# annikabrundyn/driving-dirty

Hardware: AMD Instinct MI355X
Metric: 6-view scenes/sec fwd+bwd, roadmap model bs=32 (higher is better)
Workload: dtype f32

## Files before the change

### driving-dirty_amd/csrc/conv3x3.hip

```cpp
#include <stdlib.h>

#include "dd_common.h"

namespace {

constexpr int EPI_BIAS_RELU_BITS = 5;
constexpr int EPI_RELU_BITS = 6;
constexpr int EPI_BIAS_STATS = 7;
constexpr int EPI_RELU_MASK_AFF = 8;
constexpr int EPI_RELU_BITS_W1 = 9;


template <int CIN, int S>
struct StripCfg {
  static constexpr int PXB = CIN * 4;
  static constexpr int CHUNKS = CIN / 4;
  static constexpr int NPX = 32 * S + 2;
  static constexpr int SLOTB = NPX * PXB;
  static constexpr int NCH = NPX * CHUNKS;
  static constexpr int NLOAD = (NCH + 63) / 64;
  static constexpr int SPILLB = (NLOAD * 64 - NCH) * 16;
  static constexpr int WAVEB = 3 * SLOTB + SPILLB;
  static constexpr int KGROUPS = (CIN == 32) ? 36 : 5;
  static constexpr int WFLOATS = KGROUPS * 64 * 4;
};

template <int CIN>
__device__ __forceinline__ int swz(int q) {
  return CIN == 32 ? ((q >> 1) & 7) : 0;
}

template <int CIN, int S>
__device__ __forceinline__ void load_row(const float* __restrict__ img, int H, int W, int iy, int gx0, int lane,
                                         f32x4 (&r)[StripCfg<CIN, S>::NLOAD]) {
  using C = StripCfg<CIN, S>;
  const bool rowok = (iy >= 0) && (iy < H);
  const __amdgpu_buffer_rsrc_t rs = dd_rsrc(img + (long)(rowok ? iy : 0) * W * CIN, rowok ? W * C::PXB : 0);
#pragma unroll
  for (int i = 0; i < C::NLOAD; ++i) {
    const int c = lane + 64 * i;
    const int q = c / C::CHUNKS, ch = c % C::CHUNKS;
    const int off = (c < C::NCH) ? ((gx0 + q) * C::PXB + ch * 16) : -16;
    r[i] = dd_bload4<DD_AUX_NT>(rs, off);
  }
}

template <int CIN, int S>
__device__ __forceinline__ void load_row_img(const float* __restrict__ img, int H, int W, int iy, int gx0, int lane,
                                             f32x4 (&r)[StripCfg<CIN, S>::NLOAD]) {
  using C = StripCfg<CIN, S>;
  const bool rowok = (iy >= 0) && (iy < H);
  const int so = rowok ? iy * W * C::PXB : 0;
  const __amdgpu_buffer_rsrc_t rs = dd_rsrc(img, rowok ? so + W * C::PXB : 0);
#pragma unroll
  for (int i = 0; i < C::NLOAD; ++i) {
    const int c = lane + 64 * i;
    const int q = c / C::CHUNKS, ch = c % C::CHUNKS;
    const int off = (c < C::NCH) ? ((gx0 + q) * C::PXB + ch * 16) : -16;
    r[i] = dd_bload4<DD_AUX_NT>(rs, off, so);
  }
}

template <int CIN, int S, bool SWZ>
__device__ __forceinline__ void store_row(char* slot, char* spill, int lane,
                                          const f32x4 (&r)[StripCfg<CIN, S>::NLOAD]) {
  using C = StripCfg<CIN, S>;
#pragma unroll
  for (int i = 0; i < C::NLOAD; ++i) {
    const int c = lane + 64 * i;
    const int q = c / C::CHUNKS, ch = c % C::CHUNKS;
    char* dst = slot + q * C::PXB + ((ch ^ (SWZ ? swz<CIN>(q) : 0)) << 4);
    if (64 * (i + 1) > C::NCH) dst = (c < C::NCH) ? dst : spill + (c - C::NCH) * 16;
    *(f32x4*)dst = r[i];
  }
}

template <int S, bool SWZ>
__device__ __forceinline__ void store_row_aff(char* slot, char* spill, int lane, const f32x4 (&r)[StripCfg<32, S>::NLOAD],
                                              bool rowok, int gx0, int W, f32x4 sc, f32x4 sh) {
  using C = StripCfg<32, S>;
#pragma unroll
  for (int i = 0; i < C::NLOAD; ++i) {
    const int c = lane + 64 * i;
    const int q = c / C::CHUNKS, ch = c % C::CHUNKS;
    char* dst = slot + q * C::PXB + ((ch ^ (SWZ ? swz<32>(q) : 0)) << 4);
    if (64 * (i + 1) > C::NCH) dst = (c < C::NCH) ? dst : spill + (c - C::NCH) * 16;
    const bool in = rowok && (gx0 + q >= 0) && (gx0 + q < W);
    f32x4 v = r[i];
    v.x = in ? fmaxf(v.x * sc.x + sh.x, 0.f) : 0.f;
    v.y = in ? fmaxf(v.y * sc.y + sh.y, 0.f) : 0.f;
    v.z = in ? fmaxf(v.z * sc.z + sh.z, 0.f) : 0.f;
    v.w = in ? fmaxf(v.w * sc.w + sh.w, 0.f) : 0.f;
    *(f32x4*)dst = v;
  }
}

template <int CIN, int S, int EPI, int WPB, bool AFF = false>
__global__ __launch_bounds__(WPB * 64) void conv_strip_fwd(const float* __restrict__ x, const float* __restrict__ wp,
                                                           const float* __restrict__ bias,
                                                           const float* __restrict__ msk, float* __restrict__ y,
                                                           unsigned* __restrict__ bits_out, int B, int H, int W, int Ho,
                                                           int Wo, int nstrips, const float* __restrict__ aff = nullptr,
                                                           float* __restrict__ stats = nullptr) {
  using C = StripCfg<CIN, S>;
  extern __shared__ __attribute__((aligned(16))) char smem[];
  const int tid = threadIdx.x;
  const int lane = tid & 63;
  const int wave = __builtin_amdgcn_readfirstlane(tid >> 6);
  {
    f32x4* wl4 = (f32x4*)smem;
    const f32x4* wg4 = (const f32x4*)wp;
    for (int i = tid; i < C::WFLOATS / 4; i += WPB * 64) wl4[i] = wg4[i];
  }
  __syncthreads();
  char* ring = smem + C::WFLOATS * 4 + wave * C::WAVEB;
  char* spill = ring + 3 * C::SLOTB;
  const char* wl = smem;
  const int h = lane >> 5, n = lane & 31;
  const float bv = (EPI == DD_EPI_BIAS || EPI == DD_EPI_BIAS_RELU || EPI == EPI_BIAS_RELU_BITS || EPI == EPI_BIAS_STATS) ? bias[n] : 0.f;
  f32x4 asc = {1.f, 1.f, 1.f, 1.f}, ash = {0.f, 0.f, 0.f, 0.f};
  if (AFF) {
// ... 70 lines not shown
#pragma unroll
        for (int jp = 0; jp < 5; ++jp) {
          const int tap = min(2 * jp + h, 8);
          const int dy = tap / 3, dx = tap - 3 * dy;
          const char* rowb = ring + ((S * yy + dy) % 3) * C::SLOTB;
          const f32x4 a = *(const f32x4*)(rowb + (S * n + dx) * 16);
          const f32x4 w = *(const f32x4*)(wl + (jp * 64 + lane) * 16);
          acc = DD_MFMA(a.x, w.x, acc);
          acc = DD_MFMA(a.y, w.y, acc);
          acc = DD_MFMA(a.z, w.z, acc);
        }
      }

#pragma unroll
      for (int s = 0; s < S; ++s) {
        const int iy = S * yy + 2 + s;
        if constexpr (AFF) store_row_aff<S, true>(ring + ((iy + 1) % 3) * C::SLOTB, spill, lane, pre[s], iy >= 0 && iy < H, gx0, W, asc, ash);
        else store_row<CIN, S, true>(ring + ((iy + 1) % 3) * C::SLOTB, spill, lane, pre[s]);
      }

      const __amdgpu_buffer_rsrc_t ys = dd_rsrc(y + orow, Wo * 128);
      unsigned sign_word = 0;
#pragma unroll
      for (int r = 0; r < 16; ++r) {
        float v = acc[r];
        if (EPI == DD_EPI_BIAS || EPI == EPI_BIAS_STATS) v += bv;
        if (EPI == EPI_BIAS_STATS && x0 + dd_acc_row(r, lane) < Wo) {
          st_sum += v;
          st_sq += v * v;
        }
        if (EPI == DD_EPI_BIAS_RELU || EPI == EPI_BIAS_RELU_BITS) v = fmaxf(v + bv, 0.f);
        if (EPI == DD_EPI_RELU_MASK) v = (mreg[r] > 0.f) ? v : 0.f;
        if (EPI == EPI_RELU_MASK_AFF) v = (mreg[r] * msc + msh > 0.f) ? v : 0.f;
        if (EPI == EPI_RELU_BITS) v = ((__builtin_bit_cast(unsigned, mreg[r]) >> n) & 1u) ? v : 0.f;
        dd_bstore1<DD_AUX_NT>(ys, ((x0 + dd_acc_row(r, lane)) * 32 + n) * 4, v);
        if (EPI == EPI_BIAS_RELU_BITS) {
          const unsigned long long m = __ballot(v > 0.f);
          const int i0 = (r & 3) + 8 * (r >> 2);
          if (n == i0) sign_word = (unsigned)m;
          if (n == i0 + 4) sign_word = (unsigned)(m >> 32);
        }
      }
      if (EPI == EPI_BIAS_RELU_BITS) {
        const __amdgpu_buffer_rsrc_t bs = dd_rsrc(bits_out + (long)(b * Ho + yy) * Wo, Wo * 4);
        __builtin_amdgcn_raw_buffer_store_b32(sign_word, bs, (h == 0) ? (x0 + n) * 4 : -16, 0, 0);
      }
    }
  }
  if (EPI == EPI_BIAS_STATS) {
    const long gwl = ((long)(blockIdx.x * WPB + wave) * 64 + lane) * 2;
    stats[gwl] = st_sum;
    stats[gwl + 1] = st_sq;
  }
}

template <int WPB, int MASK>
__global__ __launch_bounds__(WPB * 64) void conv_s2_dgrad(const float* __restrict__ dy, const float* __restrict__ wp,
                                                          const float* __restrict__ msk, float* __restrict__ dx,
                                                          int B, int H, int W, int Ho, int Wo, int nstrips,
                                                          const float* __restrict__ aff = nullptr) {
  using C = StripCfg<32, 1>;
  extern __shared__ __attribute__((aligned(16))) char smem[];
  const int tid = threadIdx.x;
  const int lane = tid & 63;
  const int wave = __builtin_amdgcn_readfirstlane(tid >> 6);
  {
    f32x4* wl4 = (f32x4*)smem;
    const f32x4* wg4 = (const f32x4*)wp;
    for (int i = tid; i < C::WFLOATS / 4; i += WPB * 64) wl4[i] = wg4[i];
  }
  __syncthreads();
  const int nr = (H + 1) / 2;
  const float msc = (MASK == 3) ? aff[64 + (lane & 31)] : 1.f, msh = (MASK == 3) ? aff[96 + (lane & 31)] : 0.f;
  char* ring = smem + C::WFLOATS * 4 + wave * C::WAVEB;
  char* spill = ring + 3 * C::SLOTB;
  const char* wl = smem;
  const int h = lane >> 5, n = lane & 31;

  long idx, end;
  dd_range((long)B * nstrips * nr, blockIdx.x * WPB + wave, gridDim.x * WPB, idx, end);
  while (idx < end) {
    const long col = idx / nr;
    const int r0 = (int)(idx - col * nr);
    const int r1 = (int)min((long)nr, r0 + (end - idx));
    idx += r1 - r0;
    const int b = (int)(col / nstrips), s0 = (int)(col % nstrips) * 32;
    const float* dyb = dy + (long)b * Ho * Wo * 32;

#pragma unroll
    for (int d = 0; d < 2; ++d) {
      f32x4 t[C::NLOAD];
      load_row<32, 1>(dyb, Ho, Wo, r0 + d, s0, lane, t);
      store_row<32, 1, true>(ring + ((r0 + d) % 3) * C::SLOTB, spill, lane, t);
    }

    for (int r = r0; r < r1; ++r) {
      f32x4 pre[C::NLOAD];
      load_row<32, 1>(dyb, Ho, Wo, r + 2, s0, lane, pre);
      __builtin_amdgcn_sched_barrier(0);

      const char* row_r = ring + (r % 3) * C::SLOTB;
      const char* row_r1 = ring + ((r + 1) % 3) * C::SLOTB;
#define DD_TILE(PY, PX, NTAP, ...)                                                              \
  {                                                                                             \
    constexpr int taps[NTAP][3] = {__VA_ARGS__};                                                \
    const int yi = 2 * r + (PY);                                                                \
// ... 113 lines not shown
      float anext[16];
      {
        const bool ok = yy + 1 < Ho;
        const __amdgpu_buffer_rsrc_t as = dd_rsrc(dyb + (long)(ok ? yy + 1 : 0) * Wo * 32, ok ? Wo * 128 : 0);
#pragma unroll
        for (int pp = 0; pp < 16; ++pp) anext[pp] = dd_bload1<DD_AUX_NT>(as, aoff + pp * 256);
      }
      __builtin_amdgcn_sched_barrier(0);

      if (CIN == 32) {
        const char* rb0 = ring + ((S * yy + 0) % 3) * C::SLOTB;
        const char* rb1 = ring + ((S * yy + 1) % 3) * C::SLOTB;
        const char* rb2 = ring + ((S * yy + 2) % 3) * C::SLOTB;
#pragma unroll
        for (int pp = 0; pp < 16; ++pp) {
          const float a = areg[pp];
          bsum += a;
          const int off = (S * (2 * pp + h)) * 128 + n * 4;
#pragma unroll
          for (int dx = 0; dx < 3; ++dx) {
            acc[0 + dx] = DD_MFMA(a, *(const float*)(rb0 + off + dx * 128), acc[0 + dx]);
            acc[3 + dx] = DD_MFMA(a, *(const float*)(rb1 + off + dx * 128), acc[3 + dx]);
            acc[6 + dx] = DD_MFMA(a, *(const float*)(rb2 + off + dx * 128), acc[6 + dx]);
          }
        }
      } else {
        const char* rb = ring + ((S * yy + dy4) % 3) * C::SLOTB + dx4 * 16 + c4 * 4;
#pragma unroll
        for (int pp = 0; pp < 16; ++pp) {
          const float a = areg[pp];
          bsum += a;
          acc[0] = DD_MFMA(a, *(const float*)(rb + (S * (2 * pp + h)) * 16), acc[0]);
        }
      }

#pragma unroll
      for (int s = 0; s < S; ++s) {
        const int iy = S * yy + 2 + s;
        if constexpr (AFF) store_row_aff<S, false>(ring + ((iy + 1) % 3) * C::SLOTB, spill, lane, pre[s], iy >= 0 && iy < H, gx0, W, asc, ash);
        else store_row<CIN, S, false>(ring + ((iy + 1) % 3) * C::SLOTB, spill, lane, pre[s]);
      }
#pragma unroll
      for (int pp = 0; pp < 16; ++pp) areg[pp] = anext[pp];
    }
  }

#pragma unroll
  for (int t = 0; t < NT; ++t)
#pragma unroll
    for (int r = 0; r < 16; ++r) part[(((long)gw * NT + t) * 16 + r) * 64 + lane] = acc[t][r];
  bpart[(long)gw * 64 + lane] = bsum;
}

template <int CIN>
__global__ __launch_bounds__(1024) void conv_wgrad_reduce(const float* __restrict__ part,
                                                          const float* __restrict__ bpart, float* __restrict__ dw,
                                                          float* __restrict__ db, int nw) {
  constexpr int NT = (CIN == 32) ? 9 : 1;
  constexpr int G = 16;
  __shared__ double red[G][64];
  const int l = threadIdx.x & 63, g = threadIdx.x >> 6;
  const int row = blockIdx.x;
  const float* src = (row < NT * 16) ? part + (long)row * 64 + l : bpart + l;
  const long stride = (row < NT * 16) ? (long)NT * 16 * 64 : 64;
  double s0 = 0.0, s1 = 0.0, s2 = 0.0, s3 = 0.0;
  int w = g;
  for (; w + 3 * G < nw; w += 4 * G) {
    s0 += (double)src[(long)w * stride];
    s1 += (double)src[(long)(w + G) * stride];
    s2 += (double)src[(long)(w + 2 * G) * stride];
    s3 += (double)src[(long)(w + 3 * G) * stride];
  }
  for (; w < nw; w += G) s0 += (double)src[(long)w * stride];
  red[g][l] = (s0 + s1) + (s2 + s3);
  __syncthreads();
  if (g != 0) return;
  double sd = 0.0;
#pragma unroll
  for (int i = 0; i < G; ++i) sd += red[i][l];
  const float s = (float)sd;
  if (row < NT * 16) {
    const int t = row >> 4, r = row & 15;
    const int o = dd_acc_row(r, l), j = l & 31;
    if (CIN == 32) {
      dw[((long)o * 32 + j) * 9 + t] = s;
    } else if (j < 27) {
      dw[((long)o * 3 + (j % 3)) * 9 + (j / 3)] = s;
    }
  } else {
    const double other = __shfl_xor(sd, 32);
    if (l < 32) db[l] = (float)(sd + other);
  }
}

__global__ void conv_pack_kernel(const float* __restrict__ w, float* __restrict__ p, int cin_real, int kind) {
  const int idx = blockIdx.x * blockDim.x + threadIdx.x;
  if (cin_real == 32) {
    if (idx >= 36 * 64 * 4) return;
    const int i = idx & 3, lane = (idx >> 2) & 63, g = idx >> 8;
    const int j = g & 3, t = g >> 2;
    const int n = lane & 31, c = 8 * j + 4 * (lane >> 5) + i;
    float v;
    if (kind == 0) v = w[((long)n * 32 + c) * 9 + t];
    else if (kind == 1) v = w[((long)c * 32 + n) * 9 + (8 - t)];
    else v = w[((long)c * 32 + n) * 9 + t];
    p[idx] = v;
  } else {
    if (idx >= 5 * 64 * 4) return;
    const int i = idx & 3, lane = (idx >> 2) & 63, jp = idx >> 8;
    const int n = lane & 31, tap = 2 * jp + (lane >> 5);
    p[idx] = (tap < 9 && i < 3) ? w[((long)n * 3 + i) * 9 + tap] : 0.f;
  }
}

constexpr int WINO_UFLOATS = 3 * 4 * 2 * 2 * 64 * 4;

__device__ __forceinline__ f32x2 pk_sub2(f32x2 a, f32x2 b) {
// ... 1314 lines not shown
    if (xx >= 1 && xx <= W && yy >= 1 && yy <= H) {
      const f32x4 g = *(const f32x4*)(dy + ((b * H + (yy - 1)) * W + (xx - 1)) * dy_cstore + dy_coff + 4 * q);
      const unsigned m = bits_pad[pp] >> (4 * q);
      o.x = (m & 1u) ? g.x : 0.f;
      o.y = (m & 2u) ? g.y : 0.f;
      o.z = (m & 4u) ? g.z : 0.f;
      o.w = (m & 8u) ? g.w : 0.f;
    }
    __builtin_nontemporal_store(o, out_pad + i);
  }
}

__global__ void relu_bwd_kernel(const f32x4* __restrict__ dy, const f32x4* __restrict__ y, f32x4* __restrict__ out,
                                long n4) {
  for (long i = (long)blockIdx.x * blockDim.x + threadIdx.x; i < n4; i += (long)gridDim.x * blockDim.x) {
    const f32x4 g = dy[i], v = y[i];
    f32x4 o;
    o.x = v.x > 0.f ? g.x : 0.f;
    o.y = v.y > 0.f ? g.y : 0.f;
    o.z = v.z > 0.f ? g.z : 0.f;
    o.w = v.w > 0.f ? g.w : 0.f;
    out[i] = o;
  }
}

int check_desc(const dd_conv_desc* d) {
  DD_REQUIRE(d != nullptr, DD_ERR_BAD_ARG, "conv: NULL descriptor");
  DD_REQUIRE(d->batch > 0 && d->height > 0 && d->width > 0, DD_ERR_BAD_ARG, "conv: non-positive size");
  DD_REQUIRE(d->ksize == 3 && d->pad == 1, DD_ERR_UNSUPPORTED, "conv: only k3 p1 is implemented (got k%d p%d)", d->ksize, d->pad);
  DD_REQUIRE(d->stride == 1 || d->stride == 2, DD_ERR_UNSUPPORTED, "conv: stride %d", d->stride);
  DD_REQUIRE(d->cout == 32, DD_ERR_UNSUPPORTED, "conv: Cout %d (only 32)", d->cout);
  DD_REQUIRE((d->cin_real == 32 && d->cin_store == 32) || (d->cin_real == 3 && d->cin_store == 4), DD_ERR_UNSUPPORTED,
             "conv: Cin %d stored as %d (supported: 32/32, 3/4)", d->cin_real, d->cin_store);
  DD_REQUIRE(!(d->cin_real == 3 && d->stride == 2), DD_ERR_UNSUPPORTED, "conv: Cin 3 with stride 2");
  DD_REQUIRE((long)d->width * 128 < (1L << 31), DD_ERR_UNSUPPORTED, "conv: row too long for a 32-bit buffer descriptor");
  return 0;
}

int resident_grid(const dd_conv_desc* d, long row_tiles, int wpb, int per_cu) {
  long blocks = (long)dd_cu_budget_internal() * per_cu;
  if (d->rows_per_task > 0) blocks = min(blocks, max(1L, row_tiles / d->rows_per_task / wpb));
  return (int)max(1L, min(blocks, (row_tiles + wpb - 1) / wpb));
}

template <int CIN, int S, int EPI, int WPB, bool AFF = false>
int launch_fwd(const float* x, const float* wp, const float* bias, const float* msk, float* y, const dd_conv_desc* d,
               hipStream_t st, unsigned* bits_out = nullptr, const float* aff = nullptr, float* stats = nullptr) {
  using C = StripCfg<CIN, S>;
  const int Ho = dd_conv_out(d->height, S), Wo = dd_conv_out(d->width, S);
  const int nstrips = (Wo + 31) / 32;
  const size_t lds = C::WFLOATS * 4 + (size_t)WPB * C::WAVEB;
  const int per_cu = (int)max((size_t)1, min((size_t)2, (size_t)(160 * 1024) / lds));
  const int grid = resident_grid(d, (long)d->batch * nstrips * Ho, WPB, per_cu);
  auto k = conv_strip_fwd<CIN, S, EPI, WPB, AFF>;
  if (int rc = dd_allow_lds((const void*)k, lds)) return rc;
  hipLaunchKernelGGL(k, dim3(grid), dim3(WPB * 64), lds, st, x, wp, bias, msk, y, bits_out, d->batch, d->height, d->width,
                     Ho, Wo, nstrips, aff, stats);
  DD_LAUNCH_CHECK("conv_strip_fwd");
  return 0;
}

template <int MASK>
int launch_s2_dgrad(const float* dy, const float* packed_dgrad, const float* relu_src, float* dx, const dd_conv_desc* d, hipStream_t st,
                    const float* aff) {
  using C = StripCfg<32, 1>;
  constexpr int WPB = 8;
  const int H = d->height, W = d->width, Ho = dd_conv_out(H, 2), Wo = dd_conv_out(W, 2);
  const int ns = (W + 1) / 2, nr = (H + 1) / 2;
  const int nstrips = (ns + 31) / 32;
  const size_t lds = C::WFLOATS * 4 + (size_t)WPB * C::WAVEB;
  const int grid = resident_grid(d, (long)d->batch * nstrips * nr, WPB, 1);
  auto k = conv_s2_dgrad<WPB, MASK>;
  if (int rc = dd_allow_lds((const void*)k, lds)) return rc;
  hipLaunchKernelGGL(k, dim3(grid), dim3(WPB * 64), lds, st, dy, packed_dgrad, relu_src, dx, d->batch, H, W, Ho, Wo, nstrips, aff);
  DD_LAUNCH_CHECK("conv_s2_dgrad");
  return 0;
}

template <int EPI>
int launch_wino2(const float* x, const float* up, const float* bias, const unsigned* bits_in, float* y, unsigned* bits_out,
                 const dd_conv_desc* d, hipStream_t st, const float* x4 = nullptr, float* w1part = nullptr, int* nw_out = nullptr) {
  using C = StripCfg<32, 1>;
  using C4 = StripCfg<4, 1>;
  constexpr int WPB = 4;
  const int nstrips = (d->width + 31) / 32;
  static const bool ring_env = getenv("DD_WINO2_RING") != nullptr;
  static const bool ring_w1 = getenv("DD_WINO2_RING_W1") != nullptr;
  const bool ring = ring_env || (EPI == EPI_RELU_BITS_W1 && ring_w1);
  DD_REQUIRE((long)d->height * d->width * 128 < (1L << 30), DD_ERR_UNSUPPORTED, "conv_wino2: image of %d x %d pixels: the kernel addresses an image with 30-bit offsets",
             d->height, d->width);
  const size_t lds = (size_t)WINO2_UFLOATS * 4 + (ring ? (size_t)WPB * (4 * C::SLOTB + C::SPILLB) : 0) +
                     (EPI == EPI_RELU_BITS_W1 ? (size_t)WPB * (4 * C4::SLOTB + C4::SPILLB) + 128 : 0);
  const int grid = resident_grid(d, (long)d->batch * nstrips * ((d->height + 1) / 2), WPB, 1);
  if (nw_out) *nw_out = grid * WPB;
  if (int rc = dd_allow_lds(ring ? (const void*)conv_wino2_fwd<EPI, WPB> : (const void*)conv_wino2r_fwd<EPI, WPB>, lds)) return rc;
  constexpr int pf_rows = 1;
  auto kring = conv_wino2_fwd<EPI, WPB>;
  auto kreg = conv_wino2r_fwd<EPI, WPB>;
  if (ring) hipLaunchKernelGGL(kring, dim3(grid), dim3(WPB * 64), lds, st, x, up, bias, bits_in, y, bits_out, d->batch, d->height, d->width, nstrips, x4, w1part);
  else hipLaunchKernelGGL(kreg, dim3(grid), dim3(WPB * 64), lds, st, x, up, bias, bits_in, y, bits_out, d->batch, d->height, d->width, nstrips, x4, w1part, pf_rows);
  DD_LAUNCH_CHECK("conv_wino2_fwd");
  return 0;
}

template <int EPI>
int launch_wino(const float* x, const float* up, const float* bias, const unsigned* bits_in, float* y, unsigned* bits_out,
// ... 105 lines not shown

int64_t dd_conv_wgrad_workspace_bytes(const dd_conv_desc* d) {
  if (check_desc(d)) return -1;
  const int nt = d->cin_real == 32 ? 9 : 1;
  const int64_t waves = 4 * (int64_t)DD_NUM_CU * 2;
  return waves * ((int64_t)nt * 1024 + 64) * 4;
}

static int conv_wgrad_impl(const float* x, const float* aff, const float* dy, float* dw_oihw, float* dbias, void* workspace,
                           int64_t workspace_bytes, const dd_conv_desc* d, void* stream);

int dd_conv_wgrad(const float* x, const float* dy, float* dw_oihw, float* dbias, void* workspace,
                  int64_t workspace_bytes, const dd_conv_desc* d, void* stream) {
  return conv_wgrad_impl(x, nullptr, dy, dw_oihw, dbias, workspace, workspace_bytes, d, stream);
}

int dd_conv_wgrad_bn(const float* pre_bn, const float* affine, const float* dy, float* dw_oihw, float* dbias, void* workspace,
                     int64_t workspace_bytes, const dd_conv_desc* d, void* stream) {
  DD_REQUIRE(affine, DD_ERR_BAD_ARG, "conv_wgrad_bn: NULL affine");
  DD_REQUIRE(d && d->cin_real == 32, DD_ERR_UNSUPPORTED, "conv_wgrad_bn: the input of a BN'd layer has 32 channels");
  return conv_wgrad_impl(pre_bn, affine, dy, dw_oihw, dbias, workspace, workspace_bytes, d, stream);
}

int64_t dd_conv_stats_floats(void) { return (int64_t)DD_NUM_CU * 2 * 8 * 64 * 2; }

int dd_conv_fwd_stats(const float* x, const float* packed_fwd, const float* bias, const float* in_affine, float* u,
                      float* stats, const dd_conv_desc* d, void* stream) {
  if (int rc = check_desc(d)) return rc;
  DD_REQUIRE(x && packed_fwd && bias && u && stats, DD_ERR_BAD_ARG, "conv_fwd_stats: NULL pointer");
  DD_REQUIRE(!(in_affine && d->cin_store == 4), DD_ERR_UNSUPPORTED, "conv_fwd_stats: the image layer has no BN'd input");
  hipStream_t st = (hipStream_t)stream;
  if (hipMemsetAsync(stats, 0, dd_conv_stats_floats() * sizeof(float), st) != hipSuccess)
    return dd_fail(DD_ERR_LAUNCH, "conv_fwd_stats: hipMemsetAsync failed");
  if (d->cin_store == 4) return launch_fwd<4, 1, EPI_BIAS_STATS, 8>(x, packed_fwd, bias, nullptr, u, d, st, nullptr, nullptr, stats);
  if (d->stride == 1)
    return in_affine ? launch_fwd<32, 1, EPI_BIAS_STATS, 8, true>(x, packed_fwd, bias, nullptr, u, d, st, nullptr, in_affine, stats)
                     : launch_fwd<32, 1, EPI_BIAS_STATS, 8, false>(x, packed_fwd, bias, nullptr, u, d, st, nullptr, nullptr, stats);
  return in_affine ? launch_fwd<32, 2, EPI_BIAS_STATS, 4, true>(x, packed_fwd, bias, nullptr, u, d, st, nullptr, in_affine, stats)
                   : launch_fwd<32, 2, EPI_BIAS_STATS, 4, false>(x, packed_fwd, bias, nullptr, u, d, st, nullptr, nullptr, stats);
}

static int conv_wgrad_impl(const float* x, const float* aff, const float* dy, float* dw_oihw, float* dbias, void* workspace,
                           int64_t workspace_bytes, const dd_conv_desc* d, void* stream) {
  if (int rc = check_desc(d)) return rc;
  DD_REQUIRE(x && dy && dw_oihw && dbias && workspace, DD_ERR_BAD_ARG, "conv_wgrad: NULL pointer");
  DD_REQUIRE(workspace_bytes >= dd_conv_wgrad_workspace_bytes(d), DD_ERR_WORKSPACE, "conv_wgrad: workspace %ld < %ld bytes",
             (long)workspace_bytes, (long)dd_conv_wgrad_workspace_bytes(d));
  hipStream_t st = (hipStream_t)stream;
  constexpr int WPB = 4;
  const int S = d->stride, H = d->height, W = d->width, Ho = dd_conv_out(H, S), Wo = dd_conv_out(W, S);
  const int nstrips = (Wo + 31) / 32;
  const int nt = d->cin_real == 32 ? 9 : 1;
  const int grid = resident_grid(d, (long)d->batch * nstrips * Ho, WPB, d->cin_store == 4 ? 2 : 1);
  const int nw = grid * WPB;
  float* part = (float*)workspace;
  float* bpart = part + (size_t)nw * nt * 1024;
#define DD_WG(CIN, SS, AFF)                                                                                         \
  {                                                                                                                 \
    auto k = conv_wgrad<CIN, SS, WPB, AFF>;                                                                         \
    const size_t lds = (size_t)WPB * StripCfg<CIN, SS>::WAVEB;                                                      \
    if (int rc = dd_allow_lds((const void*)k, lds)) return rc;                                                      \
    hipLaunchKernelGGL(k, dim3(grid), dim3(WPB * 64), lds, st, x, dy, part, bpart, d->batch, H, W, Ho, Wo, nstrips, \
                       aff);                                                                                        \
  }
  if (d->cin_store == 4) DD_WG(4, 1, false)
  else if (S == 1 && aff) DD_WG(32, 1, true)
  else if (S == 1) DD_WG(32, 1, false)
  else if (aff) DD_WG(32, 2, true)
  else DD_WG(32, 2, false)
#undef DD_WG
  DD_LAUNCH_CHECK("conv_wgrad");
  if (d->cin_store == 4)
    hipLaunchKernelGGL(conv_wgrad_reduce<4>, dim3(nt * 16 + 1), dim3(1024), 0, st, part, bpart, dw_oihw, dbias, nw);
  else
    hipLaunchKernelGGL(conv_wgrad_reduce<32>, dim3(nt * 16 + 1), dim3(1024), 0, st, part, bpart, dw_oihw, dbias, nw);
  DD_LAUNCH_CHECK("conv_wgrad_reduce");
  return 0;
}

int dd_relu_bwd(const float* dy, const float* y, float* out, int64_t n, void* stream) {
  DD_REQUIRE(dy && y && out && n > 0, DD_ERR_BAD_ARG, "relu_bwd: bad argument");
  DD_REQUIRE(n % 4 == 0, DD_ERR_UNSUPPORTED, "relu_bwd: n %% 4 != 0");
  const long n4 = n / 4;
  const int grid = (int)min((n4 + 255) / 256, (long)DD_NUM_CU * 8);
  hipLaunchKernelGGL(relu_bwd_kernel, dim3(grid), dim3(256), 0, (hipStream_t)stream, (const f32x4*)dy, (const f32x4*)y,
                     (f32x4*)out, n4);
  DD_LAUNCH_CHECK("relu_bwd");
  return 0;
}

int dd_relu_sign_bits(const float* x, uint32_t* bits, int64_t npix, void* stream) {
  DD_REQUIRE(x && bits && npix > 0, DD_ERR_BAD_ARG, "relu_sign_bits: bad argument");
  const long waves = (npix + 63) / 64;
  const int grid = (int)min((waves + 3) / 4, (long)DD_NUM_CU * 8);
  hipLaunchKernelGGL(relu_sign_bits_kernel, dim3(grid), dim3(256), 0, (hipStream_t)stream, x, bits, (long)npix);
  DD_LAUNCH_CHECK("relu_sign_bits");
  return 0;
}

int dd_relu_bwd_pad_bits(const float* dy, const uint32_t* bits_pad, float* out_pad, int32_t batch, int32_t h, int32_t w, int32_t dy_cstore,
                         int32_t dy_coff, void* stream) {
  DD_REQUIRE(dy && bits_pad && out_pad && batch > 0 && h > 0 && w > 0, DD_ERR_BAD_ARG, "relu_bwd_pad_bits: bad argument");
  DD_REQUIRE(dy_cstore >= 32 && dy_cstore % 4 == 0 && dy_coff >= 0 && dy_coff % 4 == 0 && dy_coff + 32 <= dy_cstore, DD_ERR_BAD_ARG,
             "relu_bwd_pad_bits: dy's 32 channels must be a 4-aligned slice of its %d stored ones (offset %d)", dy_cstore, dy_coff);
  DD_REQUIRE((((uintptr_t)dy | (uintptr_t)out_pad) & 15) == 0, DD_ERR_BAD_ARG, "relu_bwd_pad_bits: dy and out_pad must be 16-byte aligned");
  const long total = (long)batch * (h + 2) * (w + 2) * 8;
  const int grid = (int)min((total + 255) / 256, (long)DD_NUM_CU * 8);
  hipLaunchKernelGGL(relu_bwd_pad_bits_kernel, dim3(grid), dim3(256), 0, (hipStream_t)stream, dy, bits_pad, (f32x4*)out_pad,
                     batch, h, w, dy_cstore, dy_coff);
  DD_LAUNCH_CHECK("relu_bwd_pad_bits");
  return 0;
}

int64_t dd_conv_wino_packed_floats(const dd_conv_desc* d) {
  if (check_desc(d)) return -1;
  if (d->cin_real != 32 || d->stride != 1) return -1;
  return WINO_UFLOATS;
}

int dd_conv_wino_pack(const float* w_oihw, float* packed, const dd_conv_desc* d, int32_t kind, void* stream) {
  if (int rc = check_desc(d)) return rc;
  DD_REQUIRE(w_oihw && packed, DD_ERR_BAD_ARG, "conv_wino_pack: NULL pointer");
  DD_REQUIRE(d->cin_real == 32 && d->stride == 1, DD_ERR_UNSUPPORTED, "conv_wino: only the 32 -> 32 stride-1 layer");
  DD_REQUIRE(kind == 0 || kind == 1, DD_ERR_BAD_ARG, "conv_wino_pack: kind %d (0 forward, 1 data gradient)", kind);
  hipLaunchKernelGGL(conv_wino_pack_kernel, dim3((WINO_UFLOATS + 255) / 256), dim3(256), 0, (hipStream_t)stream, w_oihw, packed, kind);
  DD_LAUNCH_CHECK("conv_wino_pack");
  return 0;
}
// ... 163 lines not shown
```

Measured before the change: 4278.

## Add specialized stride-2 conv forward and wgrad kernels with software-pipelined LDS ring

Adds dedicated stride-2, 32-channel forward and weight-gradient kernels. Each keeps a 3-row LDS ring, prefetches the next two input rows, and interleaves their LDS stores with MFMA work using explicit scheduling group barriers. The forward path defers each row's output store into the next iteration. The wgrad kernel reduces its four waves' partial sums in LDS, pairing waves with atomic adds, before writing one partial per block. This cuts workspace traffic and the work left for the reduce kernel. The cost is added code complexity and a size guard on the buffer offset range.

Result: no change. 4317, median of 6 (+0.9%).

```diff
diff --git a/driving-dirty_amd/csrc/conv3x3.hip b/driving-dirty_amd/csrc/conv3x3.hip
--- a/driving-dirty_amd/csrc/conv3x3.hip
+++ b/driving-dirty_amd/csrc/conv3x3.hip
@@ -1,4 +1,6 @@
 #include <stdlib.h>
+
+#include <type_traits>
 
 #include "dd_common.h"
 
@@ -67,6 +69,21 @@
   using C = StripCfg<CIN, S>;
 #pragma unroll
   for (int i = 0; i < C::NLOAD; ++i) {
+    const int c = lane + 64 * i;
+    const int q = c / C::CHUNKS, ch = c % C::CHUNKS;
+    char* dst = slot + q * C::PXB + ((ch ^ (SWZ ? swz<CIN>(q) : 0)) << 4);
+    if (64 * (i + 1) > C::NCH) dst = (c < C::NCH) ? dst : spill + (c - C::NCH) * 16;
+    *(f32x4*)dst = r[i];
+  }
+}
+
+template <int CIN, int S, bool SWZ, int K>
+__device__ __forceinline__ void store_row_part(char* slot, char* spill, int lane, const f32x4 (&r)[StripCfg<CIN, S>::NLOAD], int part) {
+  using C = StripCfg<CIN, S>;
+#pragma unroll
+  for (int k = 0; k < K; ++k) {
+    const int i = K * part + k;
+    if (i >= C::NLOAD) continue;
     const int c = lane + 64 * i;
     const int q = c / C::CHUNKS, ch = c % C::CHUNKS;
     char* dst = slot + q * C::PXB + ((ch ^ (SWZ ? swz<CIN>(q) : 0)) << 4);
@@ -243,6 +260,168 @@
     stats[gwl] = st_sum;
     stats[gwl + 1] = st_sq;
   }
+}
+
+template <int EPI, int WPB>
+__global__ __launch_bounds__(WPB * 64) void conv_s2_fwd(const float* __restrict__ x, const float* __restrict__ wp,
+                                                        const float* __restrict__ bias, float* __restrict__ y,
+                                                        unsigned* __restrict__ bits_out, int B, int H, int W, int Ho, int Wo,
+                                                        int nstrips) {
+  using C = StripCfg<32, 2>;
+  static_assert(EPI == DD_EPI_NONE || EPI == DD_EPI_BIAS || EPI == DD_EPI_BIAS_RELU || EPI == EPI_BIAS_RELU_BITS, "conv_s2_fwd: epilogue");
+  extern __shared__ __attribute__((aligned(16))) char smem[];
+  const int tid = threadIdx.x;
+  const int lane = tid & 63;
+  const int wave = __builtin_amdgcn_readfirstlane(tid >> 6);
+  {
+    f32x4* wl4 = (f32x4*)smem;
+    const f32x4* wg4 = (const f32x4*)wp;
+    for (int i = tid; i < C::WFLOATS / 4; i += WPB * 64) wl4[i] = wg4[i];
+  }
+  __syncthreads();
+  char* ring = smem + C::WFLOATS * 4 + wave * C::WAVEB;
+  char* spill = ring + 3 * C::SLOTB;
+  const char* wl = smem;
+  const int h = lane >> 5, n = lane & 31;
+  const float bv = (EPI != DD_EPI_NONE) ? bias[n] : 0.f;
+  constexpr int FAR = 1 << 30;
+  const int pitch = W * 128, opitch = Wo * 128;
+
+  float pend[16];
+#pragma unroll
+  for (int r = 0; r < 16; ++r) pend[r] = 0.f;
+  unsigned pword = 0;
+  const float* py = y;
+  const unsigned* pb = bits_out;
+  int pso = 0, prec = 0, pvoff = 0, pbso = 0, pbrec = 0, pbvoff = 0;
+  auto store_pending = [&]() {
+    const __amdgpu_buffer_rsrc_t ys = dd_rsrc(py, prec);
+#pragma unroll
+    for (int r = 0; r < 16; ++r) dd_bstore<DD_AUX_NT>(ys, pvoff + dd_acc_row_half(r, 0) * 128, pend[r], pso);
+    if (EPI == EPI_BIAS_RELU_BITS) __builtin_amdgcn_raw_buffer_store_b32(pword, dd_rsrc(pb, pbrec), pbvoff, pbso, 0);
+  };
+
+  long idx, end;
+  dd_range((long)B * nstrips * Ho, blockIdx.x * WPB + wave, gridDim.x * WPB, idx, end);
+  while (idx < end) {
+    const long col = idx / Ho;
+    const int y0 = (int)(idx - col * Ho);
+    const int y1 = (int)min((long)Ho, y0 + (end - idx));
+    idx += y1 - y0;
+    const int b = (int)(col / nstrips), x0 = (int)(col % nstrips) * 32;
+    const float* xb = x + (long)b * H * W * 32;
+    const float* yb = y + (long)b * Ho * Wo * 32;
+    const unsigned* bob = bits_out + (EPI == EPI_BIAS_RELU_BITS ? (long)b * Ho * Wo : 0);
+    const int gx0 = 2 * x0 - 1;
+    const __amdgpu_buffer_rsrc_t xrs = dd_rsrc(xb, H * pitch);
+    int xoff[C::NLOAD];
+#pragma unroll
+    for (int i = 0; i < C::NLOAD; ++i) {
+      const int c = lane + 64 * i;
+      const int q = c / C::CHUNKS, ch = c % C::CHUNKS;
+      xoff[i] = (c < C::NCH && gx0 + q >= 0 && gx0 + q < W) ? (gx0 + q) * C::PXB + ch * 16 : FAR;
+    }
+    auto load_x = [&](int iy, f32x4 (&r)[C::NLOAD]) {
+      const int so = iy * pitch;
+#pragma unroll
+      for (int i = 0; i < C::NLOAD; ++i) r[i] = dd_bload4<DD_AUX_NT>(xrs, xoff[i], so);
+    };
+    auto read_group = [&](int g, int s0, f32x4& a, f32x4& w) {
+      const int j = g & 3, t = g >> 2, dy = t / 3, dx = t - 3 * dy;
+      int s = s0 + dy;
+      s = s >= 3 ? s - 3 : s;
+      const int q = 2 * n + dx;
+      a = *(const f32x4*)(ring + s * C::SLOTB + q * 128 + (((2 * j + h) ^ swz<32>(q)) << 4));
+      w = *(const f32x4*)(wl + ((t * 4 + j) * 64 + lane) * 16);
+    };
+
+#pragma unroll
+    for (int d = 0; d < 3; ++d) {
+      f32x4 t[C::NLOAD];
+      const int iy = 2 * y0 - 1 + d;
+      load_x(iy, t);
+      store_row<32, 2, true>(ring + d * C::SLOTB, spill, lane, t);
+    }
+    f32x4 av[2], wv[2];
+    read_group(0, 0, av[0], wv[0]);
+
+    auto row = [&](int yy, auto S0) {
+      constexpr int s0 = decltype(S0)::value;
+      constexpr int s1 = s0 == 2 ? 0 : s0 + 1, s2 = s1 == 2 ? 0 : s1 + 1;
+      __builtin_amdgcn_sched_barrier(0);
+      f32x4 pre[2][C::NLOAD];
+      load_x(2 * yy + 2, pre[0]);
+      load_x(2 * yy + 3, pre[1]);
+      store_pending();
+
+      f32x16 acc;
+#pragma unroll
+      for (int r = 0; r < 16; ++r) acc[r] = 0.f;
+#pragma unroll
+      for (int g = 0; g < 36; ++g) {
+        if (g + 1 < 36) read_group(g + 1, s0, av[(g + 1) & 1], wv[(g + 1) & 1]);
+        else read_group(0, s2, av[0], wv[0]);
+        if (g >= 24 && g < 27) store_row_part<32, 2, true, 3>(ring + s0 * C::SLOTB, spill, lane, pre[0], g - 24);
+        if (g >= 32 && g < 35) store_row_part<32, 2, true, 3>(ring + s1 * C::SLOTB, spill, lane, pre[1], g - 32);
+        const f32x4 a = av[g & 1], w = wv[g & 1];
+        acc = DD_MFMA(a.x, w.x, acc);
+        acc = DD_MFMA(a.y, w.y, acc);
+        acc = DD_MFMA(a.z, w.z, acc);
+        acc = DD_MFMA(a.w, w.w, acc);
+      }
+#pragma unroll
+      for (int g = 0; g < 36; ++g) {
+        __builtin_amdgcn_sched_group_barrier(0x008, 1, 0);
+        __builtin_amdgcn_sched_group_barrier(0x100, 2, 0);
+        __builtin_amdgcn_sched_group_barrier(0x010, 1, 0);
+        __builtin_amdgcn_sched_group_barrier(0x008, 1, 0);
+        __builtin_amdgcn_sched_group_barrier(0x010, 1, 0);
+        __builtin_amdgcn_sched_group_barrier(0x200, 1, 0);
+        __builtin_amdgcn_sched_group_barrier(0x008, 1, 0);
+        __builtin_amdgcn_sched_group_barrier(0x010, 1, 0);
+        __builtin_amdgcn_sched_group_barrier(0x200, 1, 0);
+        __builtin_amdgcn_sched_group_barrier(0x008, 1, 0);
+        __builtin_amdgcn_sched_group_barrier(0x010, 1, 0);
+        __builtin_amdgcn_sched_group_barrier(0x200, 1, 0);
+      }
+      __builtin_amdgcn_sched_barrier(0);
+
+      unsigned sign_word = 0;
+#pragma unroll
+      for (int r = 0; r < 16; ++r) {
+        float v = acc[r];
+        if (EPI == DD_EPI_BIAS) v += bv;
+        if (EPI == DD_EPI_BIAS_RELU || EPI == EPI_BIAS_RELU_BITS) v = fmaxf(v + bv, 0.f);
+        pend[r] = v;
+        if (EPI == EPI_BIAS_RELU_BITS) {
+          const unsigned long long m = __ballot(v > 0.f);
+          const int i0 = (r & 3) + 8 * (r >> 2);
+          if (n == i0) sign_word = (unsigned)m;
+          if (n == i0 + 4) sign_word = (unsigned)(m >> 32);
+        }
+      }
+      py = yb;
+      pso = yy * opitch;
+      prec = pso + opitch;
+      pvoff = ((x0 + 4 * h) * 32 + n) * 4;
+      if (EPI == EPI_BIAS_RELU_BITS) {
+        pword = sign_word;
+        pb = bob;
+        pbso = yy * Wo * 4;
+        pbrec = pbso + Wo * 4;
+        pbvoff = (h == 0) ? (x0 + n) * 4 : FAR;
+      }
+    };
+    for (int yy = y0;;) {
+      row(yy, std::integral_constant<int, 0>());
+      if (++yy >= y1) break;
+      row(yy, std::integral_constant<int, 2>());
+      if (++yy >= y1) break;
+      row(yy, std::integral_constant<int, 1>());
+      if (++yy >= y1) break;
+    }
+  }
+  store_pending();
 }
 
 template <int WPB, int MASK>
@@ -462,10 +641,170 @@
   bpart[(long)gw * 64 + lane] = bsum;
 }
 
+template <int WPB>
+__global__ __launch_bounds__(WPB * 64) void conv_s2_wgrad(const float* __restrict__ x, const float* __restrict__ dy,
+                                                          float* __restrict__ part, float* __restrict__ bpart, int B, int H,
+                                                          int W, int Ho, int Wo, int nstrips) {
+  using C = StripCfg<32, 2>;
+  static_assert(WPB == 4, "conv_s2_wgrad: the in-LDS reduction is written for four waves");
+  constexpr int NT = 9;
+  constexpr int STAGEF = NT * 1024;
+  static_assert(2 * STAGEF * 4 <= WPB * C::WAVEB, "conv_s2_wgrad: the staging areas lie over the rings");
+  extern __shared__ __attribute__((aligned(16))) char smem[];
+  const int tid = threadIdx.x;
+  const int lane = tid & 63;
+  const int wave = __builtin_amdgcn_readfirstlane(tid >> 6);
+  char* ring = smem + wave * C::WAVEB;
+  char* spill = ring + 3 * C::SLOTB;
+  const int h = lane >> 5, n = lane & 31;
+  constexpr int FAR = 1 << 30;
+  const int pitch = W * 128, opitch = Wo * 128;
+
+  int rbo_lane = h * 256 + n * 4 + 128;
+  asm("" : "+v"(rbo_lane));
+  const char* rbe = ring + h * 256 + n * 4;
+  const char* rbo = ring + rbo_lane;
+
+  f32x16 acc[NT];
+#pragma unroll
+  for (int t = 0; t < NT; ++t)
+#pragma unroll
+    for (int r = 0; r < 16; ++r) acc[t][r] = 0.f;
+  float bsum = 0.f;
+
+  long idx, end;
+  dd_range((long)B * nstrips * Ho, blockIdx.x * WPB + wave, gridDim.x * WPB, idx, end);
+  while (idx < end) {
+    const long col = idx / Ho;
+    const int y0 = (int)(idx - col * Ho);
+    const int y1 = (int)min((long)Ho, y0 + (end - idx));
+    idx += y1 - y0;
+    const int b = (int)(col / nstrips), x0 = (int)(col % nstrips) * 32;
+    const float* xb = x + (long)b * H * W * 32;
+    const float* dyb = dy + (long)b * Ho * Wo * 32;
+    const int gx0 = 2 * x0 - 1;
+    const int aoff = ((x0 + h) * 32 + n) * 4;
+    const __amdgpu_buffer_rsrc_t xrs = dd_rsrc(xb, H * pitch);
+    int xoff[C::NLOAD];
+#pragma unroll
+    for (int i = 0; i < C::NLOAD; ++i) {
+      const int c = lane + 64 * i;
+      const int q = c / C::CHUNKS, ch = c % C::CHUNKS;
+      xoff[i] = (c < C::NCH && gx0 + q >= 0 && gx0 + q < W) ? (gx0 + q) * C::PXB + ch * 16 : FAR;
+    }
+    auto load_x = [&](int iy, f32x4 (&r)[C::NLOAD]) {
+      const int so = iy * pitch;
+#pragma unroll
+      for (int i = 0; i < C::NLOAD; ++i) r[i] = dd_bload4<DD_AUX_NT>(xrs, xoff[i], so);
+    };
+    const __amdgpu_buffer_rsrc_t ars = dd_rsrc(dyb, Ho * opitch);
+    int aoffs[16];
+#pragma unroll
+    for (int pp = 0; pp < 16; ++pp) aoffs[pp] = (x0 + 2 * pp + h < Wo) ? aoff + pp * 256 : FAR;
+    auto load_dy = [&](int oy, float (&a)[16]) {
+      const int so = oy * opitch;
+#pragma unroll
+      for (int pp = 0; pp < 16; ++pp) a[pp] = dd_bload1<DD_AUX_NT>(ars, aoffs[pp], so);
+    };
+    auto read_group = [&](int g, int s0, float (&bq)[3]) {
+      const int dy = g >> 4, pp = g & 15;
+      int s = s0 + dy;
+      s = s >= 3 ? s - 3 : s;
+      const int off = s * C::SLOTB + pp * 512;
+      bq[0] = *(const float*)(rbe + off);
+      bq[1] = *(const float*)(rbo + off);
+      bq[2] = *(const float*)(rbe + off + 256);
+    };
+
+#pragma unroll
+    for (int d = 0; d < 3; ++d) {
+      f32x4 t[C::NLOAD];
+      const int iy = 2 * y0 - 1 + d;
+      load_x(iy, t);
+      store_row<32, 2, false>(ring + d * C::SLOTB, spill, lane, t);
+    }
+    float areg[16];
+    load_dy(y0, areg);
+    float bq[2][3];
+    read_group(0, 0, bq[0]);
+
+    auto row = [&](int yy, auto S0) {
+      constexpr int s0 = decltype(S0)::value;
+      constexpr int s1 = s0 == 2 ? 0 : s0 + 1, s2 = s1 == 2 ? 0 : s1 + 1;
+      __builtin_amdgcn_sched_barrier(0);
+      f32x4 pre[2][C::NLOAD];
+      load_x(2 * yy + 2, pre[0]);
+      load_x(2 * yy + 3, pre[1]);
+      float anext[16];
+      load_dy(yy + 1, anext);
+#pragma unroll
+      for (int g = 0; g < 48; ++g) {
+        const int dy = g >> 4, pp = g & 15;
+        if (g + 1 < 48) read_group(g + 1, s0, bq[(g + 1) & 1]);
+        else read_group(0, s2, bq[0]);
+        if (g >= 30 && g < 39) store_row_part<32, 2, false, 1>(ring + s0 * C::SLOTB, spill, lane, pre[0], g - 30);
+        if (g >= 39) store_row_part<32, 2, false, 1>(ring + s1 * C::SLOTB, spill, lane, pre[1], g - 39);
+        const float a = areg[pp];
+        if (dy == 0) bsum += a;
+#pragma unroll
+        for (int dx = 0; dx < 3; ++dx) acc[dy * 3 + dx] = DD_MFMA(a, bq[g & 1][dx], acc[dy * 3 + dx]);
+      }
+#pragma unroll
+      for (int g = 0; g < 48; ++g) {
+        __builtin_amdgcn_sched_group_barrier(0x008, 1, 0);
+        __builtin_amdgcn_sched_group_barrier(0x100, 3, 0);
+        __builtin_amdgcn_sched_group_barrier(0x020, 1, 0);
+        __builtin_amdgcn_sched_group_barrier(0x008, 1, 0);
+        __builtin_amdgcn_sched_group_barrier(0x020, 1, 0);
+        __builtin_amdgcn_sched_group_barrier(0x200, 1, 0);
+        __builtin_amdgcn_sched_group_barrier(0x008, 1, 0);
+        __builtin_amdgcn_sched_group_barrier(0x020, 1, 0);
+      }
+      __builtin_amdgcn_sched_barrier(0);
+#pragma unroll
+      for (int pp = 0; pp < 16; ++pp) areg[pp] = anext[pp];
+    };
+    for (int yy = y0;;) {
+      row(yy, std::integral_constant<int, 0>());
+      if (++yy >= y1) break;
+      row(yy, std::integral_constant<int, 2>());
+      if (++yy >= y1) break;
+      row(yy, std::integral_constant<int, 1>());
+      if (++yy >= y1) break;
+    }
+  }
+
+  const int lane_e = dd_fresh_lane();
+  float* stage = (float*)smem + (wave >> 1) * STAGEF + lane_e;
+  __syncthreads();
+  if (wave & 1) {
+#pragma unroll
+    for (int t = 0; t < NT; ++t)
+#pragma unroll
+      for (int r = 0; r < 16; ++r) stage[(t * 16 + r) * 64] = acc[t][r];
+  }
+  __syncthreads();
+  if (!(wave & 1)) {
+#pragma unroll
+    for (int t = 0; t < NT; ++t)
+#pragma unroll
+      for (int r = 0; r < 16; ++r) __hip_atomic_fetch_add(stage + (t * 16 + r) * 64, acc[t][r], __ATOMIC_RELAXED, __HIP_MEMORY_SCOPE_WORKGROUP);
+  }
+  __syncthreads();
+  {
+    const f32x4* sa = (const f32x4*)smem;
+    const f32x4* sb = sa + STAGEF / 4;
+    const int tid_e = lane_e + 64 * wave;
+    f32x4* out = (f32x4*)(part + (long)blockIdx.x * NT * 1024);
+    for (int i = tid_e; i < NT * 256; i += WPB * 64) out[i] = sa[i] + sb[i];
+  }
+  bpart[((long)blockIdx.x * WPB + wave) * 64 + lane_e] = bsum;
+}
+
 template <int CIN>
 __global__ __launch_bounds__(1024) void conv_wgrad_reduce(const float* __restrict__ part,
                                                           const float* __restrict__ bpart, float* __restrict__ dw,
-                                                          float* __restrict__ db, int nw) {
+                                                          float* __restrict__ db, int nw_w, int nw_b) {
   constexpr int NT = (CIN == 32) ? 9 : 1;
   constexpr int G = 16;
   __shared__ double red[G][64];
@@ -473,6 +812,7 @@
   const int row = blockIdx.x;
   const float* src = (row < NT * 16) ? part + (long)row * 64 + l : bpart + l;
   const long stride = (row < NT * 16) ? (long)NT * 16 * 64 : 64;
+  const int nw = (row < NT * 16) ? nw_w : nw_b;
   double s0 = 0.0, s1 = 0.0, s2 = 0.0, s3 = 0.0;
   int w = g;
   for (; w + 3 * G < nw; w += 4 * G) {
@@ -1893,6 +2233,15 @@
   const size_t lds = C::WFLOATS * 4 + (size_t)WPB * C::WAVEB;
   const int per_cu = (int)max((size_t)1, min((size_t)2, (size_t)(160 * 1024) / lds));
   const int grid = resident_grid(d, (long)d->batch * nstrips * Ho, WPB, per_cu);
+  if constexpr (CIN == 32 && S == 2 && !AFF && (EPI == DD_EPI_NONE || EPI == DD_EPI_BIAS || EPI == DD_EPI_BIAS_RELU || EPI == EPI_BIAS_RELU_BITS)) {
+    if ((long)d->height * d->width * 128 < (1L << 30)) {
+      auto k2 = conv_s2_fwd<EPI, WPB>;
+      if (int rc = dd_allow_lds((const void*)k2, lds)) return rc;
+      hipLaunchKernelGGL(k2, dim3(grid), dim3(WPB * 64), lds, st, x, wp, bias, y, bits_out, d->batch, d->height, d->width, Ho, Wo, nstrips);
+      DD_LAUNCH_CHECK("conv_s2_fwd");
+      return 0;
+    }
+  }
   auto k = conv_strip_fwd<CIN, S, EPI, WPB, AFF>;
   if (int rc = dd_allow_lds((const void*)k, lds)) return rc;
   hipLaunchKernelGGL(k, dim3(grid), dim3(WPB * 64), lds, st, x, wp, bias, msk, y, bits_out, d->batch, d->height, d->width,
@@ -2104,7 +2453,8 @@
   const int nstrips = (Wo + 31) / 32;
   const int nt = d->cin_real == 32 ? 9 : 1;
   const int grid = resident_grid(d, (long)d->batch * nstrips * Ho, WPB, d->cin_store == 4 ? 2 : 1);
-  const int nw = grid * WPB;
+  const bool s2 = d->cin_store == 32 && S == 2 && !aff && (long)H * W * 128 < (1L << 30);
+  const int nw = s2 ? grid : grid * WPB;
   float* part = (float*)workspace;
   float* bpart = part + (size_t)nw * nt * 1024;
 #define DD_WG(CIN, SS, AFF)                                                                                         \
@@ -2119,13 +2469,19 @@
   else if (S == 1 && aff) DD_WG(32, 1, true)
   else if (S == 1) DD_WG(32, 1, false)
   else if (aff) DD_WG(32, 2, true)
-  else DD_WG(32, 2, false)
+  else if (!s2) DD_WG(32, 2, false)
+  else {
+    auto k = conv_s2_wgrad<WPB>;
+    const size_t lds = (size_t)WPB * StripCfg<32, 2>::WAVEB;
+    if (int rc = dd_allow_lds((const void*)k, lds)) return rc;
+    hipLaunchKernelGGL(k, dim3(grid), dim3(WPB * 64), lds, st, x, dy, part, bpart, d->batch, H, W, Ho, Wo, nstrips);
+  }
 #undef DD_WG
   DD_LAUNCH_CHECK("conv_wgrad");
   if (d->cin_store == 4)
-    hipLaunchKernelGGL(conv_wgrad_reduce<4>, dim3(nt * 16 + 1), dim3(1024), 0, st, part, bpart, dw_oihw, dbias, nw);
+    hipLaunchKernelGGL(conv_wgrad_reduce<4>, dim3(nt * 16 + 1), dim3(1024), 0, st, part, bpart, dw_oihw, dbias, nw, grid * WPB);
   else
-    hipLaunchKernelGGL(conv_wgrad_reduce<32>, dim3(nt * 16 + 1), dim3(1024), 0, st, part, bpart, dw_oihw, dbias, nw);
+    hipLaunchKernelGGL(conv_wgrad_reduce<32>, dim3(nt * 16 + 1), dim3(1024), 0, st, part, bpart, dw_oihw, dbias, nw, grid * WPB);
   DD_LAUNCH_CHECK("conv_wgrad_reduce");
   return 0;
 }
```
